# karfly/learnable-triangulation-pytorch

Measured on NVIDIA H100. Metric: volumetric samples/sec (4-view 384x384, 64^3 grid), higher is better.
Workload: dtype fp16x3 (split-fp16 operands, 3 wgmma products per term, fp32 accumulate)

## Files before the change

learnable-triangulation-pytorch_b200/csrc/common.cuh:

```cuda
#pragma once
#include <cuda_runtime.h>
#include <cuda_fp16.h>
#include <stdint.h>
#include <stdio.h>
#include <stdarg.h>
#include "../../include/lt_b200.h"

namespace lt {

char* err_buf();
int fail(int code, const char* fmt, ...);

#define LT_REQUIRE(cond, ...)                                   \
  do {                                                          \
    if (!(cond)) return ::lt::fail(LT_ERR_INVALID, __VA_ARGS__); \
  } while (0)

#define LT_CHECK_LAUNCH(name)                                                                  \
  do {                                                                                         \
    cudaError_t e__ = cudaGetLastError();                                                      \
    if (e__ != cudaSuccess) return ::lt::fail(LT_ERR_CUDA, "%s: %s", name, cudaGetErrorString(e__)); \
  } while (0)

const lt_options& opts();
int sm_count();

struct DeviceOnce {
  unsigned long long done = 0;
  bool first() {
    int dev = 0;
    if (cudaGetDevice(&dev) != cudaSuccess || dev < 0 || dev > 63) return true;
    const unsigned long long bit = 1ull << dev;
    return (__atomic_fetch_or(&done, bit, __ATOMIC_ACQ_REL) & bit) == 0;
  }
};

static inline int ceil_div(long a, long b) { return (int)((a + b - 1) / b); }

typedef __half sh_t;
constexpr float kLoScale = 1.0f;
constexpr float kLoInv = 1.0f;

__device__ __forceinline__ void split_s32(float x, sh_t& hi, sh_t& lo) {
  if (fabsf(x) <= 3.402823466e+38f) x = fminf(fmaxf(x, -65504.0f), 65504.0f);
  hi = __float2half_rn(x);
  lo = __float2half_rn((x - __half2float(hi)) * kLoScale);
}
__device__ __forceinline__ float join_s32(sh_t hi, sh_t lo) {
  return fmaf(__half2float(lo), kLoInv, __half2float(hi));
}
__device__ __host__ __forceinline__ int s32_off(int c) { return ((c >> 5) << 6) + (c & 31); }

__device__ __forceinline__ void store_s32x4(sh_t* row, int c, float4 v) {
  sh_t h[4], l[4];
  split_s32(v.x, h[0], l[0]);
  split_s32(v.y, h[1], l[1]);
  split_s32(v.z, h[2], l[2]);
  split_s32(v.w, h[3], l[3]);
  sh_t* p = row + s32_off(c);
  *reinterpret_cast<uint2*>(p) = *reinterpret_cast<uint2*>(h);
// ... 36 lines not shown
```

learnable-triangulation-pytorch_b200/csrc/conv_fold.cu:

```cuda
#include "tc_common.cuh"
#include "conv_tc_params.cuh"

namespace lt {

constexpr int kFoldThreads = 384;
constexpr int kFoldSmem = 227 * 1024;

template <int NC>
struct LinesCfg {
  static constexpr int N = 3 * NC;
  static constexpr int SLICE = N * 128;
  static constexpr int B_BYTES = 9 * SLICE;
  static constexpr int PLANE = 32 * 1024;
  static constexpr int RING = 3;
  static constexpr int XCH = 2 * 2 * 4 * 2 * 4 * (NC / 4) * 4;
  static constexpr int SLAB = 8 * 1024;
  static constexpr int A_OFF = B_BYTES;
  static constexpr int S_OFF = A_OFF + RING * PLANE;
  static constexpr int X_OFF = S_OFF + 2 * SLAB;
  static constexpr int BAR_OFF = X_OFF + XCH;
  static constexpr size_t SMEM = (size_t)BAR_OFF + 128 + 1024;
  static_assert(SLICE % 1024 == 0 && B_BYTES % 1024 == 0, "B slices must start on 1024-byte swizzle atoms");
  static_assert(SMEM <= (size_t)kFoldSmem, "shared memory");
};
// ... 67 lines not shown
  uint64_t* afull = reinterpret_cast<uint64_t*>(smem + C::BAR_OFF);
  uint64_t* aempty = afull + C::RING;
  uint64_t* bfull = aempty + C::RING;
  uint64_t* rfull = bfull + 1;
  uint64_t* rempty = rfull + 2;

  const int wg = __shfl_sync(0xffffffffu, (int)(threadIdx.x >> 7), 0);
  const int lane = threadIdx.x & 31;
  const int W = p.bw, LPB = p.bh / 2;
  const long total = (long)p.N * p.th * p.OD;
  const long q0 = (long)blockIdx.x * total / gridDim.x, q1 = (long)(blockIdx.x + 1) * total / gridDim.x;

  if (threadIdx.x == 0) {
    for (int s = 0; s < C::RING; ++s) { mbar_init(&afull[s], 1); mbar_init(&aempty[s], 256); }
    mbar_init(&bfull[0], 1);
    for (int s = 0; s < 2; ++s) { mbar_init(&rfull[s], 1); mbar_init(&rempty[s], 1); }
    fence_barrier_init();
    prefetch_tmap(&tmA);
    prefetch_tmap(&tmB);
    prefetch_tmap(&tmO);
    if (p.residual != LT_RES_NONE) prefetch_tmap(&tmR);
  }
  __syncthreads();

  if (wg == 0) {
    regs_release_producer();
    if (threadIdx.x < 32) {
      if (elect_one()) {
        mbar_expect_tx(&bfull[0], (uint32_t)C::B_BYTES);
        tma_load_3d(bsm, &tmB, &bfull[0], 0, 0, 0);
      }
      const uint32_t box_bytes = (uint32_t)((p.bh + 2) * W * 128), res_bytes = (uint32_t)(LPB * W * 128);
      int s = 0;
      uint32_t ph = 0, rph = 0;
      long q = q0;
      LinesPiece pc;
      while (lines_next_piece(p, q, q1, pc)) {
        for (int dd = pc.dA - 1; dd <= pc.dB; ++dd) {
          mbar_wait(&aempty[s], ph ^ 1u);
          if (elect_one()) {
            mbar_expect_tx(&afull[s], box_bytes);
            tma_load_5d(asm_ + (size_t)s * C::PLANE, &tmA, &afull[s], 0, 0, pc.h0 - 1, dd, pc.n);
          }
          __syncwarp();
          if (++s == C::RING) { s = 0; ph ^= 1u; }
          if (dd > pc.dA) {
            for (int r = 0; r < 2; ++r) {
              mbar_wait(&rempty[r], rph ^ 1u);
              if (elect_one()) {
                if (p.residual != LT_RES_NONE) {
                  mbar_expect_tx(&rfull[r], res_bytes);
                  tma_load_5d(ssm + (size_t)r * C::SLAB, &tmR, &rfull[r], 0, 0, pc.h0 + r * LPB, dd - 1, pc.n);
                } else {
                  mbar_arrive_local(&rfull[r]);
// ... 169 lines not shown
  int rc = make_in_map(&tmA, d, p.bw, p.bh + 2, 1, 1, in);
  if (rc) return rc;
  const uint64_t dims[3] = {64, (uint64_t)C::N, 9};
  const uint64_t str[2] = {128, (uint64_t)C::SLICE};
  const uint32_t bx[3] = {64, (uint32_t)C::N, 9};
  rc = make_map(&tmB, weight, 3, dims, str, bx, nullptr, 1);
  if (rc) return rc;
  CUtensorMap tmO, tmR;
  const int f32 = d->out_format == LT_FMT_F32;
  const uint64_t odims[5] = {(uint64_t)(f32 ? 32 : 64), (uint64_t)d->OW, (uint64_t)d->OH, (uint64_t)d->OD, (uint64_t)d->N};
  const uint64_t ostr[4] = {128, 128ull * d->OW, 128ull * d->OW * d->OH, 128ull * d->OW * d->OH * d->OD};
  const uint32_t obx[5] = {(uint32_t)(f32 ? 32 : 64), (uint32_t)d->OW, (uint32_t)(p.bh / 2), 1, 1};
  rc = make_map(&tmO, out, 5, odims, ostr, obx, nullptr, 1, f32);
  if (rc) return rc;
  rc = make_map(&tmR, residual ? residual : out, 5, odims, ostr, obx, nullptr, 1, f32);
  if (rc) return rc;
  static DeviceOnce configured;
  if (configured.first()) {
    cudaError_t e = cudaFuncSetAttribute(conv_lines_kernel<NC>, cudaFuncAttributeMaxDynamicSharedMemorySize, kFoldSmem);
    if (e != cudaSuccess) return fail(LT_ERR_CUDA, "conv_lines: cudaFuncSetAttribute: %s", cudaGetErrorString(e));
  }
  const long planes = (long)p.N * p.th * p.OD;
  const int grid = (int)(planes < sm_count() ? planes : sm_count());
  conv_lines_kernel<NC><<<grid, kFoldThreads, C::SMEM, st>>>(tmA, tmB, tmO, tmR, p);
  cudaError_t e = cudaGetLastError();
  if (e != cudaSuccess) return fail(LT_ERR_CUDA, "conv_lines_kernel: %s", cudaGetErrorString(e));
  return LT_OK;
}

template <int K, int NC>
struct FoldCfg {
  static_assert(K == 7, "the 3^3 layers run on conv_lines_kernel");
  static constexpr int BW = 8, BH = 16, BD = 2;
  static constexpr int WBOX = BW + K - 1, HBOX = BH + K - 1, DBOX = BD;
  static constexpr int A_BYTES = WBOX * HBOX * DBOX * 128;
  static constexpr int ASTAGES = K;
  static constexpr int TAP = NC * 128;
  static constexpr int B_SLICE = K * TAP;
  static constexpr int MB = 2;
  static constexpr int AVAIL = kFoldSmem - 1024 - 256;
  static constexpr int ARING = 2;
  static constexpr int BRING_FIT = (AVAIL - ARING * A_BYTES) / B_SLICE;
  static constexpr int BRING = BRING_FIT > 4 ? 4 : BRING_FIT;
  static constexpr int A_OFF = BRING * B_SLICE;
  static constexpr int BAR_OFF = A_OFF + ARING * A_BYTES;
  static constexpr size_t SMEM = (size_t)BAR_OFF + 256 + 1024;
  static_assert(BW * BH * BD == 256 && BH % 8 == 0, "two m64 blocks of whole 8-wide lines per warpgroup");
  static_assert(A_BYTES % 1024 == 0 && B_SLICE % 1024 == 0, "boxes must start on 1024-byte swizzle atoms");
// ... 35 lines not shown
                                                                    const __grid_constant__ CUtensorMap tmB, const TcParams p) {
  using C = FoldCfg<K, NC>;
  extern __shared__ uint8_t smem_raw[];
  uint8_t* smem = reinterpret_cast<uint8_t*>((reinterpret_cast<uintptr_t>(smem_raw) + 1023) & ~(uintptr_t)1023);
  uint8_t* bsm = smem;
  uint8_t* asm_ = smem + C::A_OFF;
  uint64_t* afull = reinterpret_cast<uint64_t*>(smem + C::BAR_OFF);
  uint64_t* aempty = afull + C::ARING;
  uint64_t* bfull = aempty + C::ARING;
  uint64_t* bempty = bfull + C::BRING;

  const int wg = __shfl_sync(0xffffffffu, (int)(threadIdx.x >> 7), 0);
  const int lane = threadIdx.x & 31;
  const int ntiles = p.tw * p.th * p.td * p.tn;

  if (threadIdx.x == 0) {
    for (int s = 0; s < C::ARING; ++s) { mbar_init(&afull[s], 1); mbar_init(&aempty[s], 256); }
    for (int s = 0; s < C::BRING; ++s) { mbar_init(&bfull[s], 1); mbar_init(&bempty[s], 2); }
    fence_barrier_init();
    prefetch_tmap(&tmA);
    prefetch_tmap(&tmB);
  }
  __syncthreads();

  if (wg == 0) {
    regs_release_producer();
    if (threadIdx.x < 32) {
      int sa = 0, sb = 0;
      uint32_t pa = 0, pb = 0;
      for (int t = blockIdx.x; t < ntiles; t += gridDim.x) {
        int ow0, oh0, od0, nb;
        fold_tile_origin(p, t, ow0, oh0, od0, nb);
        for (int as = 0; as < C::ASTAGES; ++as) {
          mbar_wait(&aempty[sa], pa ^ 1u);
          if (elect_one()) {
            mbar_expect_tx(&afull[sa], (uint32_t)C::A_BYTES);
            tma_load_5d(asm_ + (size_t)sa * C::A_BYTES, &tmA, &afull[sa], 0, ow0 - K / 2, oh0 - K / 2, od0 + as - K / 2, nb);
          }
          __syncwarp();
          if (++sa == C::ARING) { sa = 0; pa ^= 1u; }
          for (int kw = 0; kw < K; ++kw) {
            mbar_wait(&bempty[sb], pb ^ 1u);
            if (elect_one()) {
              mbar_expect_tx(&bfull[sb], (uint32_t)C::B_SLICE);
              tma_load_3d(bsm + (size_t)sb * C::B_SLICE, &tmB, &bfull[sb], 0, 0, (kw * K + as) * K);
            }
            __syncwarp();
            if (++sb == C::BRING) { sb = 0; pb ^= 1u; }
          }
        }
      }
    }
    return;
  }

  regs_claim_consumer();
  const int g = wg - 1, warp = (threadIdx.x >> 5) & 3;
  float d1[C::MB][NC / 2], d2[C::MB][NC / 2];
#pragma unroll
  for (int b = 0; b < C::MB; ++b)
#pragma unroll
    for (int i = 0; i < NC / 2; ++i) { d1[b][i] = 0.f; d2[b][i] = 0.f; }
  int blk_dd[C::MB], blk_hb[C::MB];
  uint32_t row0[C::MB];
#pragma unroll
  for (int b = 0; b < C::MB; ++b) {
    const int blk = C::MB * g + b;
    blk_dd[b] = blk / (C::BH / 8);
    blk_hb[b] = blk % (C::BH / 8);
    row0[b] = (uint32_t)((blk_dd[b] * C::HBOX + blk_hb[b] * 8 + 2 * warp) * C::WBOX + (lane & 7));
  }
  const uint32_t mlane = (uint32_t)(lane >> 3);
  const int r_lo = warp * 16 + (lane >> 2);
  const int c2 = 2 * (lane & 3);
  const uint32_t bsm0 = smem_u32(bsm), asm0 = smem_u32(asm_);
  const bool wg_lead = (threadIdx.x & 127) == 0;
  int bprev = -1;
  for (int kt = 0;; ++kt) {
    const int t = blockIdx.x + kt * gridDim.x;
    if (t >= ntiles) break;
#pragma unroll 1
    for (int as = 0; as < C::ASTAGES; ++as) {
      const int na = kt * C::ASTAGES + as;
      const int sa = na % C::ARING;
      mbar_wait(&afull[sa], (uint32_t)(na / C::ARING) & 1u);
      const uint32_t box = asm0 + (uint32_t)(sa * C::A_BYTES);
#pragma unroll 1
      for (int kw = 0; kw < K; ++kw) {
        const int nbs = na * K + kw;
        const int sb = nbs % C::BRING;
        mbar_wait(&bfull[sb], (uint32_t)(nbs / C::BRING) & 1u);
        const uint32_t bslice = bsm0 + (uint32_t)(sb * C::B_SLICE);
        uint32_t ln[K + 1][C::MB][2][4];
#pragma unroll
        for (int b = 0; b < C::MB; ++b) fold_load_line(ln[0][b], box, row0[b] + kw, mlane);
#pragma unroll
        for (int kh = 0; kh < K; ++kh) {
#pragma unroll
          for (int b = 0; b < C::MB; ++b) fold_load_line(ln[kh + 1][b], box, row0[b] + kw + (uint32_t)((kh + 1) * C::WBOX), mlane);
          wg_fence();
          const uint64_t bd = make_sw128_desc(bslice + (uint32_t)(kh * C::TAP));
          const uint32_t acc = (as == 0 && kw == 0 && kh == 0) ? 0u : 1u;
#pragma unroll
// ... 40 lines not shown
                         const void* residual, void* out, cudaStream_t st) {
  constexpr int K = 7;
  using C = FoldCfg<K, NC>;
  TcParams p;
  fill_params(d, p, 1, NC, NC, 3, scale, shift, residual, out);
  p.bw = C::BW; p.bh = C::BH; p.bd = C::BD; p.bn = 1;
  p.tw = ceil_div(d->OW, p.bw); p.th = ceil_div(d->OH, p.bh); p.td = ceil_div(d->OD, p.bd); p.tn = d->N;
  p.stages = C::ARING;
  CUtensorMap tmA, tmB;
  int rc = make_in_map(&tmA, d, C::WBOX, C::HBOX, C::DBOX, 1, in);
  if (rc) return rc;
  const uint64_t dims[3] = {64, (uint64_t)NC, (uint64_t)K * K * K};
  const uint64_t str[2] = {128, (uint64_t)NC * 128};
  const uint32_t bx[3] = {64, (uint32_t)NC, (uint32_t)K};
  rc = make_map(&tmB, weight, 3, dims, str, bx, nullptr, 1);
  if (rc) return rc;
  static DeviceOnce configured;
  if (configured.first()) {
    cudaError_t e = cudaFuncSetAttribute(conv_fold_kernel<K, NC>, cudaFuncAttributeMaxDynamicSharedMemorySize, kFoldSmem);
    if (e != cudaSuccess) return fail(LT_ERR_CUDA, "conv_fold: cudaFuncSetAttribute: %s", cudaGetErrorString(e));
  }
  const long ntiles = (long)p.tw * p.th * p.td * p.tn;
  const int grid = (int)(ntiles < sm_count() ? ntiles : sm_count());
  conv_fold_kernel<K, NC><<<grid, kFoldThreads, C::SMEM, st>>>(tmA, tmB, p);
  cudaError_t e = cudaGetLastError();
  if (e != cudaSuccess) return fail(LT_ERR_CUDA, "conv_fold_kernel: %s", cudaGetErrorString(e));
  return LT_OK;
}

int conv_fold_supported(const lt_conv_desc* d) {
  const bool cubic = d->KD == d->KH && d->KH == d->KW && (d->KW == 3 || d->KW == 7);
  const int pd = d->KW / 2;
  return cubic && d->Cin == 32 && d->Cout <= 32 && d->sd == 1 && d->sh == 1 && d->sw == 1 && d->pd == pd && d->ph == pd &&
         d->pw == pd && d->OD == d->ID && d->OH == d->IH && d->OW == d->IW && d->osd == 1 && d->osh == 1 && d->osw == 1 &&
         d->ood == 0 && d->ooh == 0 && d->oow == 0 && d->FD == d->OD && d->FH == d->OH && d->FW == d->OW && d->FC == 32 &&
         d->in_format == LT_FMT_S32 && d->IW >= 16 && (d->KW == 7 || d->IW <= 64);
}

int conv_fold_fwd(const lt_conv_desc* d, const void* in, const void* weight, const float* scale, const float* shift,
                  const void* residual, void* out, void* stream) {
  LT_REQUIRE(conv_fold_supported(d), "conv_fold: unsupported layer shape");
  const cudaStream_t st = (cudaStream_t)stream;
  const bool narrow = d->Cout <= 16;
  if (d->KW == 3)
    return narrow ? conv_lines_run<16>(d, in, weight, scale, shift, residual, out, st)
                  : conv_lines_run<32>(d, in, weight, scale, shift, residual, out, st);
  return narrow ? conv_fold_run<16>(d, in, weight, scale, shift, residual, out, st)
                : conv_fold_run<32>(d, in, weight, scale, shift, residual, out, st);
// ... 42 lines not shown
```

learnable-triangulation-pytorch_b200/csrc/conv_tail.cu:

```cuda
#include "conv_tc_params.cuh"
#include "softargmax_common.cuh"

namespace lt {

struct TailParams {
  const float* scale1; const float* shift1;
  const float* scale2; const float* shift2;
  const float* scale3; const float* bias3;
  float* logits;
  long rows;
  long tiles;
  int FC;
  const float* coord;
  float* partial;
  int B, J, tiles_per_sample, softmax;
  float mult;
};

constexpr int kTailThreads = 384;
constexpr int kTailStages = 2;
constexpr int kTailWBytes = 32 * 128;
constexpr int kTailHBytes = 64 * 128;
constexpr int kTailOffH = kTailStages * kATileBytes;
constexpr int kTailOffW = kTailOffH + 2 * kTailHBytes;
// ... 44 lines not shown
  }
}

template <int STATS>
__global__ void __launch_bounds__(kTailThreads, 2) v2v_tail_kernel(const __grid_constant__ CUtensorMap tmX,
                                                                    const __grid_constant__ CUtensorMap tmW1,
                                                                    const __grid_constant__ CUtensorMap tmW2,
                                                                    const __grid_constant__ CUtensorMap tmW3, const TailParams p) {
  extern __shared__ uint8_t smem_raw[];
  uint8_t* smem = reinterpret_cast<uint8_t*>((reinterpret_cast<uintptr_t>(smem_raw) + 1023) & ~(uintptr_t)1023);
  uint8_t* w_tiles = smem + kTailOffW;
  uint64_t* a_full = reinterpret_cast<uint64_t*>(smem + kTailOffBar);
  uint64_t* a_empty = a_full + kTailStages;
  uint64_t* w_full = a_empty + kTailStages;

  const int wg = __shfl_sync(0xffffffffu, (int)(threadIdx.x >> 7), 0);
  const int lane = threadIdx.x & 31;
  if (threadIdx.x == 0) {
    for (int s = 0; s < kTailStages; ++s) { mbar_init(&a_full[s], 1); mbar_init(&a_empty[s], 2); }
    mbar_init(w_full, 1);
    fence_barrier_init();
  }
  __syncthreads();

  if (wg == 0) {
    if (threadIdx.x < 32) {
      if (elect_one()) {
        prefetch_tmap(&tmX);
        mbar_expect_tx(w_full, 3u * kTailWBytes);
        tma_load_2d(w_tiles, &tmW1, w_full, 0, 0);
        tma_load_2d(w_tiles + kTailWBytes, &tmW2, w_full, 0, 0);
        tma_load_2d(w_tiles + 2 * kTailWBytes, &tmW3, w_full, 0, 0);
      }
      __syncwarp();
      uint32_t s = 0, ph = 0;
      for (long t = blockIdx.x; t < p.tiles; t += gridDim.x) {
        mbar_wait(&a_empty[s], ph ^ 1u);
        if (elect_one()) {
          mbar_expect_tx(&a_full[s], (uint32_t)kATileBytes);
          tma_load_2d(smem + s * kATileBytes, &tmX, &a_full[s], 0, (int)(t * 128));
        }
        __syncwarp();
        if (++s == kTailStages) { s = 0; ph ^= 1u; }
      }
    }
    return;
  }

  const int g = wg - 1;
  const int wq = (threadIdx.x >> 5) & 3;
  const int rl = wq * 16 + (lane >> 2);
  const int c2 = 2 * (lane & 3);
  const uint32_t hbase = smem_u32(smem + kTailOffH + g * kTailHBytes);
  const uint64_t hd = make_sw128_desc(hbase);
  const uint64_t w1 = make_sw128_desc(smem_u32(w_tiles)), w2 = make_sw128_desc(smem_u32(w_tiles + kTailWBytes)),
                 w3 = make_sw128_desc(smem_u32(w_tiles + 2 * kTailWBytes));
  constexpr bool SM = STATS == 1;
// ... 17 lines not shown
        SoftState t{o[0], o[1], o[2], o[3], o[4]};
        st_merge(a, t, SM);
      }
      float* dst = p.partial + (((long)b * gridDim.x + blockIdx.x) * p.J + lane) * 5;
      dst[0] = a.m; dst[1] = a.d; dst[2] = a.sx; dst[3] = a.sy; dst[4] = a.sz;
    }
    tail_consumers_sync();
  };
  if (STATS) {
    for (int i = threadIdx.x - 128; i < p.B * p.J; i += 256) {
      const int b = i / p.J, j = i % p.J;
      const long lo = (long)b * p.tiles_per_sample, G = gridDim.x;
      const long f0 = lo + (((long)blockIdx.x - lo) % G + G) % G;
      if (!(f0 < lo + p.tiles_per_sample)) {
        float* dst = p.partial + (((long)b * G + blockIdx.x) * p.J + j) * 5;
        dst[0] = SM ? -INFINITY : 0.0f; dst[1] = 0.f; dst[2] = 0.f; dst[3] = 0.f; dst[4] = 0.f;
      }
    }
  }

  mbar_wait(w_full, 0);
  uint32_t s = 0, ph = 0;
  for (long t = blockIdx.x; t < p.tiles; t += gridDim.x) {
    if (STATS) {
      const int b = (int)(t / p.tiles_per_sample);
      if (b != cur_b) {
        if (cur_b >= 0) flush(cur_b);
        cur_b = b;
      }
    }
    float d[16];
    mbar_wait(&a_full[s], ph);
    gemm32(d, make_sw128_desc(smem_u32(smem + s * kATileBytes + g * kTailHBytes)), w1);
    if ((threadIdx.x & 127) == 0) mbar_arrive_local(&a_empty[s]);
    if (++s == kTailStages) { s = 0; ph ^= 1u; }
#pragma unroll
    for (int layer = 0; layer < 2; ++layer) {
      tail_wg_sync(g);
      hidden_store(d, layer == 0 ? p.scale1 : p.scale2, layer == 0 ? p.shift1 : p.shift2, hbase, rl, c2);
      fence_proxy_async();
      tail_wg_sync(g);
      gemm32(d, hd, layer == 0 ? w2 : w3);
    }
#pragma unroll
    for (int h = 0; h < 2; ++h) {
      const int rw = (lane >> 2) + 8 * h;
// ... 50 lines not shown
    if (rc) return rc;
  }
  const void* ws[3] = {w1, w2, w3};
  const uint64_t wrows[3] = {32, 32, (uint64_t)((p.FC + 15) & ~15)};
  for (int i = 0; i < 3; ++i) {
    const uint64_t dims[2] = {64, wrows[i]};
    const uint64_t str[1] = {128};
    const uint32_t bx[2] = {64, 32};
    int rc = make_map(&tmW[i], ws[i], 2, dims, str, bx, nullptr, 1);
    if (rc) return rc;
  }
  p.tiles = (p.rows + 127) / 128;
  static DeviceOnce configured;
  if (configured.first()) {
    cudaError_t e = cudaFuncSetAttribute(v2v_tail_kernel<0>, cudaFuncAttributeMaxDynamicSharedMemorySize, kTailSmem);
    if (e == cudaSuccess) e = cudaFuncSetAttribute(v2v_tail_kernel<1>, cudaFuncAttributeMaxDynamicSharedMemorySize, kTailSmemStats);
    if (e == cudaSuccess) e = cudaFuncSetAttribute(v2v_tail_kernel<2>, cudaFuncAttributeMaxDynamicSharedMemorySize, kTailSmemStats);
    if (e != cudaSuccess) return fail(LT_ERR_CUDA, "v2v_tail: cudaFuncSetAttribute: %s", cudaGetErrorString(e));
  }
  long grid = 2L * sm_count();
  if (grid > p.tiles) grid = p.tiles;
  if (grid_out) *grid_out = (int)grid;
  cudaStream_t st = (cudaStream_t)stream;
  if (stats == 1) v2v_tail_kernel<1><<<(unsigned)grid, kTailThreads, kTailSmemStats, st>>>(tmX, tmW[0], tmW[1], tmW[2], p);
  else if (stats == 2) v2v_tail_kernel<2><<<(unsigned)grid, kTailThreads, kTailSmemStats, st>>>(tmX, tmW[0], tmW[1], tmW[2], p);
  else v2v_tail_kernel<0><<<(unsigned)grid, kTailThreads, kTailSmem, st>>>(tmX, tmW[0], tmW[1], tmW[2], p);
  LT_CHECK_LAUNCH("v2v_tail_kernel");
  return LT_OK;
}

extern "C" int lt_v2v_tail_fwd(const void* x, const void* w1, const void* w2, const void* w3, const float* scale1, const float* shift1,
                               const float* scale2, const float* shift2, const float* scale3, const float* bias3, float* logits, long rows,
                               int FC, void* stream) {
  LT_REQUIRE(x && w1 && w2 && w3 && scale1 && shift1 && scale2 && shift2 && scale3 && bias3 && logits, "v2v_tail: null pointer");
  LT_REQUIRE(rows > 0 && rows < (1L << 31) && FC % 4 == 0 && FC >= 4 && FC <= 32, "v2v_tail: bad sizes (rows=%ld FC=%d)", rows, FC);
  TailParams p;
  p.scale1 = scale1; p.shift1 = shift1; p.scale2 = scale2; p.shift2 = shift2; p.scale3 = scale3; p.bias3 = bias3;
  p.logits = logits; p.rows = rows; p.FC = FC;
  p.coord = nullptr; p.partial = nullptr; p.B = 0; p.J = 0; p.tiles_per_sample = 1; p.softmax = 0; p.mult = 1.0f;
  return launch_tail(x, w1, w2, w3, p, 0, nullptr, stream);
}

extern "C" int lt_v2v_tail_stats_fwd(const void* x, const void* w1, const void* w2, const void* w3, const float* scale1, const float* shift1,
                                     const float* scale2, const float* shift2, const float* scale3, const float* bias3, float* logits, int B,
                                     long nvox, int FC, const float* coord, int J, float multiplier, int softmax, void* workspace,
                                     size_t workspace_bytes, int* n_partials, void* stream) {
  LT_REQUIRE(x && w1 && w2 && w3 && scale1 && shift1 && scale2 && shift2 && scale3 && bias3 && logits && coord && workspace && n_partials,
             "v2v_tail_stats: null pointer");
  LT_REQUIRE(B > 0 && nvox > 0 && nvox % 128 == 0 && (long)B * nvox < (1L << 31), "v2v_tail_stats: bad sizes (B=%d nvox=%ld)", B, nvox);
  LT_REQUIRE(FC % 4 == 0 && FC >= 4 && FC <= kTailStatMaxFC && J > 0 && J <= FC, "v2v_tail_stats: need J <= FC <= %d, FC %% 4 == 0", kTailStatMaxFC);
// ... 12 lines not shown
```

learnable-triangulation-pytorch_b200/csrc/conv_tc.cu:

```cuda
#include "tc_common.cuh"
#include "conv_tc_params.cuh"
#include <stdlib.h>
#include <string.h>

namespace lt {

constexpr int kTcThreads = 384;

struct TcUnit {
  int m, n0, z, q_begin, nchunks;
};
__device__ __forceinline__ TcUnit tc_unit(const TcParams& p, int u, int m_tiles, int nchunks_all) {
  TcUnit w;
  const int n = u % p.n_tiles;
  u /= p.n_tiles;
  w.m = u % m_tiles;
  w.z = u / m_tiles;
  w.n0 = n * p.Nt;
  w.q_begin = (int)(((long)w.z * nchunks_all) / p.splits);
  w.nchunks = (int)(((long)(w.z + 1) * nchunks_all) / p.splits) - w.q_begin;
  return w;
}
__device__ __forceinline__ void tc_tile_origin(const TcParams& p, int t, int& ow0, int& oh0, int& od0, int& nb0) {
  ow0 = (t % p.tw) * p.bw; t /= p.tw;
// ... 25 lines not shown
  const int epi_bytes = tc_epi_bytes(NT, p.splits);
  const bool staged = epi_bytes > 0;
  uint8_t* ebuf = smem + (size_t)p.stages * kStage;
  uint64_t* full = reinterpret_cast<uint64_t*>(ebuf + epi_bytes);
  uint64_t* empty = full + p.stages;
  uint64_t* efull = empty + p.stages;
  uint64_t* edone = efull + 1;

  const int wg = __shfl_sync(0xffffffffu, (int)(threadIdx.x >> 7), 0);
  const int lane = threadIdx.x & 31;
  const int m_tiles = p.tw * p.th * p.td * p.tn;
  const int units = m_tiles * p.n_tiles * p.splits;
  const int nchunks_all = p.KD * p.KH * p.KW * p.CB;

  if (threadIdx.x == 0) {
    for (int s = 0; s < p.stages; ++s) { mbar_init(&full[s], 1); mbar_init(&empty[s], 2); }
    mbar_init(efull, 1);
    mbar_init(edone, 256);
    fence_barrier_init();
    prefetch_tmap(&tmA);
    prefetch_tmap(&tmB);
  }
  __syncthreads();

  if (wg == 0) {
    regs_release_producer();
    if (staged && threadIdx.x == 32) {
      uint32_t eph = 0;
      for (int u = blockIdx.x; u < units; u += gridDim.x) {
        const TcUnit w = tc_unit(p, u, m_tiles, nchunks_all);
        int ow0, oh0, od0, nb0;
        tc_tile_origin(p, w.m, ow0, oh0, od0, nb0);
        bulk_wait_read0();
        if (p.residual != LT_RES_NONE) {
          mbar_expect_tx(efull, (uint32_t)epi_bytes);
          for (int sl = 0; sl < NT / 32; ++sl) {
            int g, c;
            epi_slab(p, w.n0 + 32 * sl, g, c);
            tma_load_5d(ebuf + sl * kSlabBytes, &tmE.res[g], efull, c, ow0, oh0, od0, nb0);
          }
        } else {
          mbar_arrive_local(efull);
        }
        mbar_wait(edone, eph);
        eph ^= 1u;
        for (int sl = 0; sl < NT / 32; ++sl) {
          int g, c;
          epi_slab(p, w.n0 + 32 * sl, g, c);
          tma_store_5d(&tmE.out[g], ebuf + sl * kSlabBytes, c, ow0, oh0, od0, nb0);
        }
        bulk_commit();
      }
      bulk_wait0();
    }
    if (threadIdx.x < 32) {
      int s = 0;
      uint32_t ph = 0;
      for (int u = blockIdx.x; u < units; u += gridDim.x) {
        const TcUnit w = tc_unit(p, u, m_tiles, nchunks_all);
        int ow0, oh0, od0, nb0;
        tc_tile_origin(p, w.m, ow0, oh0, od0, nb0);
        int tap = w.q_begin / p.CB, cb = w.q_begin - tap * p.CB;
        int kw = tap % p.KW, kh = (tap / p.KW) % p.KH, kd = tap / (p.KW * p.KH);
        const int ax = ow0 * p.sw - p.pw, ay = oh0 * p.sh - p.ph, az = od0 * p.sd - p.pd, bn0 = w.n0 * p.b_nmul;
        for (int q = 0, qa = w.q_begin; q < w.nchunks; ++q, ++qa) {
          mbar_wait(&empty[s], ph ^ 1u);
          uint8_t* a_dst = smem + (size_t)s * kStage;
          if (elect_one()) {
            mbar_expect_tx(&full[s], (uint32_t)kStage);
            tma_load_5d(a_dst, &tmA, &full[s], cb * 64, ax + kw, ay + kh, az + kd, nb0);
            tma_load_2d(a_dst + kATileBytes, &tmB, &full[s], qa * p.b_step0, qa * p.b_step1 + bn0);
          }
          __syncwarp();
          if (++cb == p.CB) { cb = 0; if (++kw == p.KW) { kw = 0; if (++kh == p.KH) { kh = 0; ++kd; } } }
          if (++s == p.stages) { s = 0; ph ^= 1u; }
        }
      }
    }
    return;
  }

  regs_claim_consumer();
  const int g = wg - 1;
  float d1[NT / 2], d2[NT / 2];
#pragma unroll
  for (int i = 0; i < NT / 2; ++i) { d1[i] = 0.f; d2[i] = 0.f; }
  const int r0 = g * 64 + ((threadIdx.x >> 5) & 3) * 16 + (lane >> 2);
  const int c2 = 2 * (lane & 3);
  const uint32_t ring0 = smem_u32(smem);
  int s = 0;
  uint32_t ph = 0, eph = 0;
  for (int u = blockIdx.x; u < units; u += gridDim.x) {
    const TcUnit w = tc_unit(p, u, m_tiles, nchunks_all);
    int prev = -1;
    for (int q = 0; q < w.nchunks; ++q) {
      mbar_wait(&full[s], ph);
      const uint32_t a_addr = ring0 + (uint32_t)(s * kStage) + (uint32_t)(g * 64 * 128);
      const uint32_t b_addr = ring0 + (uint32_t)(s * kStage) + kATileBytes;
      const uint64_t ad = make_sw128_desc(a_addr), bd = make_sw128_desc(b_addr);
      const uint32_t acc = (q == 0) ? 0u : 1u;
      wg_fence();
      if (p.terms == 3) {
        wgmma_f16<NT>(d1, ad, bd, acc);
        wgmma_f16<NT>(d1, ad + 2, bd + 2, 1u);
        wgmma_f16<NT>(d2, ad, bd + 4, acc);
        wgmma_f16<NT>(d2, ad + 2, bd + 6, 1u);
        wgmma_f16<NT>(d2, ad + 4, bd, 1u);
        wgmma_f16<NT>(d2, ad + 6, bd + 2, 1u);
      } else if (p.terms == 1) {
        wgmma_f16<NT>(d1, ad, bd, acc);
        wgmma_f16<NT>(d1, ad + 2, bd + 2, 1u);
      } else {
        wgmma_f16<NT>(d1, ad, bd, acc);
        wgmma_f16<NT>(d1, ad + 2, bd + 2, 1u);
        wgmma_f16<NT>(d1, ad + 4, bd + 4, 1u);
// ... 165 lines not shown
  slot.used = true;
  slot.key = key;
  slot.map = *map;
  return LT_OK;
}

static int pow2_ceil(int v) { int p = 1; while (p < v) p <<= 1; return p; }

static void pick_box(int OW, int OH, int OD, int N, int* box) {
  double best = 1e300;
  for (int bw = 1; bw <= 128; bw <<= 1)
    for (int bh = 1; bw * bh <= 128; bh <<= 1)
      for (int bd = 1; bw * bh * bd <= 128; bd <<= 1) {
        const int bn = 128 / (bw * bh * bd);
        if (bw > pow2_ceil(OW) || bh > pow2_ceil(OH) || bd > pow2_ceil(OD) || bn > pow2_ceil(N)) continue;
        const double padded = (double)ceil_div(OW, bw) * bw * ceil_div(OH, bh) * bh * (double)ceil_div(OD, bd) * bd * ceil_div(N, bn) * bn;
        const double score = padded * (1.0 + 1e-3 / bw);
        if (score < best) { best = score; box[0] = bw; box[1] = bh; box[2] = bd; box[3] = bn; }
      }
  if (best == 1e300) { box[0] = pow2_ceil(OW) > 128 ? 128 : pow2_ceil(OW); box[1] = box[2] = 1; box[3] = 128 / box[0]; }
}

__global__ void __launch_bounds__(256) splitk_reduce_kernel(const TcParams p, long m_tiles, int coutp) {
  const int c4 = coutp >> 2;
  const long total = m_tiles * 128 * c4;
  for (long i = (long)blockIdx.x * blockDim.x + threadIdx.x; i < total; i += (long)gridDim.x * blockDim.x) {
    const int co = (int)(i % c4) * 4;
    const long tr = i / c4;
    const int row = (int)(tr % 128);
    long t = tr / 128;
    const int twi = (int)(t % p.tw); t /= p.tw;
    const int thi = (int)(t % p.th); t /= p.th;
    const int tdi = (int)(t % p.td); t /= p.td;
    const int tni = (int)t;
    int r_ = row;
    const int dw = r_ % p.bw; r_ /= p.bw;
    const int dh = r_ % p.bh; r_ /= p.bh;
    const int dd = r_ % p.bd; r_ /= p.bd;
    const int ow = twi * p.bw + dw, oh = thi * p.bh + dh, od = tdi * p.bd + dd, nb = tni * p.bn + r_;
    if (!(ow < p.OW && oh < p.OH && od < p.OD && nb < p.N) || co >= p.FC) continue;
    const long opix = (((long)nb * p.FD + (od * p.osd + p.ood)) * p.FH + (oh * p.osh + p.ooh)) * p.FW + (ow * p.osw + p.oow);
    float4 a = make_float4(0.f, 0.f, 0.f, 0.f);
    for (int z = 0; z < p.splits; ++z) {
      const float4 v = *reinterpret_cast<const float4*>(p.ws + ((size_t)z * m_tiles * 128 + tr) * p.ws_ld + co);
      a.x += v.x; a.y += v.y; a.z += v.z; a.w += v.w;
    }
// ... 13 lines not shown
    else store_s32x4(reinterpret_cast<sh_t*>(p.out) + opix * 2 * p.FC, co, o);
  }
}

static int out_groups(const lt_conv_desc* d) {
  const int g = (d->ogd > 1 ? d->ogd : 1) * (d->ogh > 1 ? d->ogh : 1) * (d->ogw > 1 ? d->ogw : 1);
  return g;
}

static int pick_nt(int CoutP) {
  for (int nt = 128; nt > 16; nt >>= 1)
    if (CoutP % nt == 0) return nt;
  return 16;
}

template <int NT>
static int launch_nt(const CUtensorMap& tmA, const CUtensorMap& tmB, const TcEpiMaps& tmE, const TcParams& p, dim3 grid, size_t smem,
                     cudaStream_t st) {
  static DeviceOnce configured;
  if (configured.first()) {
    cudaError_t e = cudaFuncSetAttribute(conv_tc_kernel<NT>, cudaFuncAttributeMaxDynamicSharedMemorySize, (int)(227 * 1024));
    if (e != cudaSuccess) return fail(LT_ERR_CUDA, "conv_tc: cudaFuncSetAttribute: %s", cudaGetErrorString(e));
  }
  conv_tc_kernel<NT><<<grid, kTcThreads, smem, st>>>(tmA, tmB, tmE, p);
  cudaError_t e = cudaGetLastError();
  if (e != cudaSuccess) return fail(LT_ERR_CUDA, "conv_tc_kernel: %s", cudaGetErrorString(e));
  return LT_OK;
}

static double tc_model_clocks(long tiles, int chunks, int nt, int splits, int sm) {
  const long units = tiles * splits;
  const long grid = units < sm ? units : sm;
  const long waves = (units + grid - 1) / grid;
  const double chunk = fmax(12.0 * 64.0 * nt / 128.0, (kATileBytes + nt * 128.0) / 30.0);
  const double epilogue = 128.0 * nt * 4.0 / 30.0;
  double t = (double)waves * ((double)ceil_div(chunks, splits) * chunk + epilogue);
  if (splits > 1) t += 7000.0 + (double)tiles * 128 * nt * 4.0 * (splits + 2) / 1500.0;
  return t;
}

static void tc_plan(long m_tiles, int n_tiles, int nt, int chunks, int terms, int n_maps, int splitk, size_t ws_bytes, int sm,
                    int* splits_out, int* grid_out) {
  const long tiles = m_tiles * n_tiles;
  int best = 1;
  if (splitk && terms != 0 && n_maps == 1) {
    const size_t per_split = (size_t)tiles * 128 * nt * sizeof(float);
    double best_t = tc_model_clocks(tiles, chunks, nt, 1, sm);
    for (int s = 2; s <= chunks / 4 && (size_t)s * per_split <= ws_bytes; ++s) {
      const double t = tc_model_clocks(tiles, chunks, nt, s, sm);
// ... 49 lines not shown
  const int epi_bytes = tc_epi_bytes(p.Nt, splits);
  int stages = (kTcSmemBudget - epi_bytes) / stage_bytes;
  if (stages > 8) stages = 8;
  p.stages = stages;
  const size_t smem = (size_t)stages * stage_bytes + epi_bytes + (2 * stages + 2) * 8 + 1024;
  TcEpiMaps tmE{};
  int rc;
  if (epi_bytes) {
    rc = make_epi_maps(p, &tmE);
    if (rc) return rc;
  }
  switch (p.Nt) {
    case 128: rc = launch_nt<128>(tmA, tmB, tmE, p, dim3(grid), smem, st); break;
    case 64: rc = launch_nt<64>(tmA, tmB, tmE, p, dim3(grid), smem, st); break;
    case 32: rc = launch_nt<32>(tmA, tmB, tmE, p, dim3(grid), smem, st); break;
    case 16: rc = launch_nt<16>(tmA, tmB, tmE, p, dim3(grid), smem, st); break;
    default: return fail(LT_ERR_INVALID, "conv_tc: unsupported N tile %d", p.Nt);
  }
  if (rc) return rc;
  if (splits > 1) {
    const long total = m_tiles * 128 * (p.ws_ld / 4);
    long blocks = (total + 255) / 256;
    if (blocks > 4L * sm_count()) blocks = 4L * sm_count();
    splitk_reduce_kernel<<<(unsigned)blocks, 256, 0, st>>>(p, m_tiles, p.ws_ld);
    cudaError_t e = cudaGetLastError();
    if (e != cudaSuccess) return fail(LT_ERR_CUDA, "splitk_reduce_kernel: %s", cudaGetErrorString(e));
  }
  return LT_OK;
}

void fill_params(const lt_conv_desc* d, TcParams& p, int CB, int CoutP, int Nt, int terms, const float* scale, const float* shift,
                        const void* residual, void* out) {
  p.OW = d->OW; p.OH = d->OH; p.OD = d->OD; p.N = d->N;
  int box[4];
  pick_box(d->OW, d->OH, d->OD, d->N, box);
  p.bw = box[0]; p.bh = box[1]; p.bd = box[2]; p.bn = box[3];
  p.tw = ceil_div(d->OW, p.bw); p.th = ceil_div(d->OH, p.bh); p.td = ceil_div(d->OD, p.bd); p.tn = ceil_div(d->N, p.bn);
  p.KW = d->KW; p.KH = d->KH; p.KD = d->KD; p.pw = d->pw; p.ph = d->ph; p.pd = d->pd;
  p.sw = d->sw; p.sh = d->sh; p.sd = d->sd;
  p.CB = CB; p.b_step0 = 0; p.b_step1 = CoutP; p.b_nmul = 1; p.Nt = Nt; p.terms = terms;
  p.FC = d->FC; p.FD = d->FD; p.FH = d->FH; p.FW = d->FW;
  p.osd = d->osd; p.osh = d->osh; p.osw = d->osw; p.ood = d->ood; p.ooh = d->ooh; p.oow = d->oow;
  p.relu = d->relu; p.residual = d->residual; p.out_format = d->out_format;
  p.scale = scale; p.shift = shift; p.res = residual; p.out = out;
  p.splits = 1; p.ws = nullptr; p.ws_ld = 0; p.ws_gain = 1.0f; p.stages = 0; p.n_tiles = 1;
  p.n_maps = out_groups(d);
  p.oc = p.n_maps > 1 ? d->Cout / p.n_maps : CoutP;
  p.gh = d->ogh > 1 ? d->ogh : 1; p.gw = d->ogw > 1 ? d->ogw : 1;
}
// ... 142 lines not shown
```

Baseline: 206.9.

## Launch conv kernels with PDL and prefetch weights before grid dependency wait

Switches the conv_lines, conv_fold, conv_tc, v2v tail and split-K reduce launches to programmatic dependent launch. Each kernel issues its weight (B) TMA loads before griddepcontrol.wait and triggers its dependents near its last tile. This lets one kernel's prologue and weight fetch overlap the previous kernel's tail, hiding launch gaps across a chain of many small conv layers. The risk is subtle barrier and transaction accounting: the producer must skip B loads that were already issued, and an early trigger could race if any dependent touches data before its wait.

```diff
diff --git a/learnable-triangulation-pytorch_b200/csrc/common.cuh b/learnable-triangulation-pytorch_b200/csrc/common.cuh
--- a/learnable-triangulation-pytorch_b200/csrc/common.cuh
+++ b/learnable-triangulation-pytorch_b200/csrc/common.cuh
@@ -4,6 +4,7 @@
 #include <stdint.h>
 #include <stdio.h>
 #include <stdarg.h>
+#include <utility>
 #include "../../include/lt_b200.h"
 
 namespace lt {
@@ -36,6 +37,29 @@
 };
 
 static inline int ceil_div(long a, long b) { return (int)((a + b - 1) / b); }
+
+__device__ __forceinline__ void pdl_wait() { asm volatile("griddepcontrol.wait;" ::: "memory"); }
+__device__ __forceinline__ void pdl_trigger() { asm volatile("griddepcontrol.launch_dependents;" ::: "memory"); }
+
+template <typename... KArgs, typename... Args>
+static inline cudaError_t launch_pdl(void (*kernel)(KArgs...), dim3 grid, dim3 block, size_t smem, cudaStream_t st, Args&&... args) {
+  cudaLaunchAttribute attr[1];
+  attr[0].id = cudaLaunchAttributeProgrammaticStreamSerialization;
+  attr[0].val.programmaticStreamSerializationAllowed = 1;
+  cudaLaunchConfig_t cfg = {};
+  cfg.gridDim = grid;
+  cfg.blockDim = block;
+  cfg.dynamicSmemBytes = smem;
+  cfg.stream = st;
+  cfg.attrs = attr;
+  cfg.numAttrs = 1;
+  return cudaLaunchKernelEx(&cfg, kernel, std::forward<Args>(args)...);
+}
+#define LT_CHECK_PDL(name, call)                                                                \
+  do {                                                                                          \
+    cudaError_t e__ = (call);                                                                   \
+    if (e__ != cudaSuccess) return ::lt::fail(LT_ERR_CUDA, "%s: %s", name, cudaGetErrorString(e__)); \
+  } while (0)
 
 typedef __half sh_t;
 constexpr float kLoScale = 1.0f;
diff --git a/learnable-triangulation-pytorch_b200/csrc/conv_fold.cu b/learnable-triangulation-pytorch_b200/csrc/conv_fold.cu
--- a/learnable-triangulation-pytorch_b200/csrc/conv_fold.cu
+++ b/learnable-triangulation-pytorch_b200/csrc/conv_fold.cu
@@ -113,14 +113,19 @@
     if (p.residual != LT_RES_NONE) prefetch_tmap(&tmR);
   }
   __syncthreads();
+  if (threadIdx.x < 32) {
+    if (elect_one()) {
+      mbar_expect_tx(&bfull[0], (uint32_t)C::B_BYTES);
+      tma_load_3d(bsm, &tmB, &bfull[0], 0, 0, 0);
+    }
+    __syncwarp();
+  }
+  pdl_wait();
+  pdl_trigger();
 
   if (wg == 0) {
     regs_release_producer();
     if (threadIdx.x < 32) {
-      if (elect_one()) {
-        mbar_expect_tx(&bfull[0], (uint32_t)C::B_BYTES);
-        tma_load_3d(bsm, &tmB, &bfull[0], 0, 0, 0);
-      }
       const uint32_t box_bytes = (uint32_t)((p.bh + 2) * W * 128), res_bytes = (uint32_t)(LPB * W * 128);
       int s = 0;
       uint32_t ph = 0, rph = 0;
@@ -336,8 +341,7 @@
   }
   const long planes = (long)p.N * p.th * p.OD;
   const int grid = (int)(planes < sm_count() ? planes : sm_count());
-  conv_lines_kernel<NC><<<grid, kFoldThreads, C::SMEM, st>>>(tmA, tmB, tmO, tmR, p);
-  cudaError_t e = cudaGetLastError();
+  cudaError_t e = launch_pdl(conv_lines_kernel<NC>, grid, dim3(kFoldThreads), C::SMEM, st, tmA, tmB, tmO, tmR, p);
   if (e != cudaSuccess) return fail(LT_ERR_CUDA, "conv_lines_kernel: %s", cudaGetErrorString(e));
   return LT_OK;
 }
@@ -419,6 +423,18 @@
     prefetch_tmap(&tmB);
   }
   __syncthreads();
+  constexpr int kBPre = C::BRING < C::ASTAGES * K ? C::BRING : C::ASTAGES * K;
+  if (threadIdx.x < 32 && (int)blockIdx.x < ntiles) {
+    if (elect_one()) {
+      for (int i = 0; i < kBPre; ++i) {
+        const int as = i / K, kw = i % K;
+        mbar_expect_tx(&bfull[i], (uint32_t)C::B_SLICE);
+        tma_load_3d(bsm + (size_t)i * C::B_SLICE, &tmB, &bfull[i], 0, 0, (kw * K + as) * K);
+      }
+    }
+    __syncwarp();
+  }
+  pdl_wait();
 
   if (wg == 0) {
     regs_release_producer();
@@ -438,7 +454,7 @@
           if (++sa == C::ARING) { sa = 0; pa ^= 1u; }
           for (int kw = 0; kw < K; ++kw) {
             mbar_wait(&bempty[sb], pb ^ 1u);
-            if (elect_one()) {
+            if (!(t == (int)blockIdx.x && as * K + kw < kBPre) && elect_one()) {
               mbar_expect_tx(&bfull[sb], (uint32_t)C::B_SLICE);
               tma_load_3d(bsm + (size_t)sb * C::B_SLICE, &tmB, &bfull[sb], 0, 0, (kw * K + as) * K);
             }
@@ -476,6 +492,7 @@
   for (int kt = 0;; ++kt) {
     const int t = blockIdx.x + kt * gridDim.x;
     if (t >= ntiles) break;
+    if (t + (int)gridDim.x >= ntiles) pdl_trigger();
 #pragma unroll 1
     for (int as = 0; as < C::ASTAGES; ++as) {
       const int na = kt * C::ASTAGES + as;
@@ -562,8 +579,7 @@
   }
   const long ntiles = (long)p.tw * p.th * p.td * p.tn;
   const int grid = (int)(ntiles < sm_count() ? ntiles : sm_count());
-  conv_fold_kernel<K, NC><<<grid, kFoldThreads, C::SMEM, st>>>(tmA, tmB, p);
-  cudaError_t e = cudaGetLastError();
+  cudaError_t e = launch_pdl(conv_fold_kernel<K, NC>, grid, dim3(kFoldThreads), C::SMEM, st, tmA, tmB, p);
   if (e != cudaSuccess) return fail(LT_ERR_CUDA, "conv_fold_kernel: %s", cudaGetErrorString(e));
   return LT_OK;
 }
diff --git a/learnable-triangulation-pytorch_b200/csrc/conv_tail.cu b/learnable-triangulation-pytorch_b200/csrc/conv_tail.cu
--- a/learnable-triangulation-pytorch_b200/csrc/conv_tail.cu
+++ b/learnable-triangulation-pytorch_b200/csrc/conv_tail.cu
@@ -90,17 +90,20 @@
     fence_barrier_init();
   }
   __syncthreads();
+  if (threadIdx.x < 32) {
+    if (elect_one()) {
+      prefetch_tmap(&tmX);
+      mbar_expect_tx(w_full, 3u * kTailWBytes);
+      tma_load_2d(w_tiles, &tmW1, w_full, 0, 0);
+      tma_load_2d(w_tiles + kTailWBytes, &tmW2, w_full, 0, 0);
+      tma_load_2d(w_tiles + 2 * kTailWBytes, &tmW3, w_full, 0, 0);
+    }
+    __syncwarp();
+  }
+  pdl_wait();
 
   if (wg == 0) {
     if (threadIdx.x < 32) {
-      if (elect_one()) {
-        prefetch_tmap(&tmX);
-        mbar_expect_tx(w_full, 3u * kTailWBytes);
-        tma_load_2d(w_tiles, &tmW1, w_full, 0, 0);
-        tma_load_2d(w_tiles + kTailWBytes, &tmW2, w_full, 0, 0);
-        tma_load_2d(w_tiles + 2 * kTailWBytes, &tmW3, w_full, 0, 0);
-      }
-      __syncwarp();
       uint32_t s = 0, ph = 0;
       for (long t = blockIdx.x; t < p.tiles; t += gridDim.x) {
         mbar_wait(&a_empty[s], ph ^ 1u);
@@ -164,6 +167,7 @@
   mbar_wait(w_full, 0);
   uint32_t s = 0, ph = 0;
   for (long t = blockIdx.x; t < p.tiles; t += gridDim.x) {
+    if (t + gridDim.x >= p.tiles) pdl_trigger();
     if (STATS) {
       const int b = (int)(t / p.tiles_per_sample);
       if (b != cur_b) {
@@ -260,10 +264,12 @@
   if (grid > p.tiles) grid = p.tiles;
   if (grid_out) *grid_out = (int)grid;
   cudaStream_t st = (cudaStream_t)stream;
-  if (stats == 1) v2v_tail_kernel<1><<<(unsigned)grid, kTailThreads, kTailSmemStats, st>>>(tmX, tmW[0], tmW[1], tmW[2], p);
-  else if (stats == 2) v2v_tail_kernel<2><<<(unsigned)grid, kTailThreads, kTailSmemStats, st>>>(tmX, tmW[0], tmW[1], tmW[2], p);
-  else v2v_tail_kernel<0><<<(unsigned)grid, kTailThreads, kTailSmem, st>>>(tmX, tmW[0], tmW[1], tmW[2], p);
-  LT_CHECK_LAUNCH("v2v_tail_kernel");
+  const dim3 g((unsigned)grid), b(kTailThreads);
+  cudaError_t e;
+  if (stats == 1) e = launch_pdl(v2v_tail_kernel<1>, g, b, kTailSmemStats, st, tmX, tmW[0], tmW[1], tmW[2], p);
+  else if (stats == 2) e = launch_pdl(v2v_tail_kernel<2>, g, b, kTailSmemStats, st, tmX, tmW[0], tmW[1], tmW[2], p);
+  else e = launch_pdl(v2v_tail_kernel<0>, g, b, kTailSmem, st, tmX, tmW[0], tmW[1], tmW[2], p);
+  LT_CHECK_PDL("v2v_tail_kernel", e);
   return LT_OK;
 }
 
diff --git a/learnable-triangulation-pytorch_b200/csrc/conv_tc.cu b/learnable-triangulation-pytorch_b200/csrc/conv_tc.cu
--- a/learnable-triangulation-pytorch_b200/csrc/conv_tc.cu
+++ b/learnable-triangulation-pytorch_b200/csrc/conv_tc.cu
@@ -71,6 +71,20 @@
     prefetch_tmap(&tmB);
   }
   __syncthreads();
+  int b_pre = 0;
+  if (threadIdx.x < 32 && (int)blockIdx.x < units) {
+    const TcUnit w = tc_unit(p, blockIdx.x, m_tiles, nchunks_all);
+    b_pre = w.nchunks < p.stages ? w.nchunks : p.stages;
+    if (elect_one()) {
+      for (int q = 0; q < b_pre; ++q) {
+        const int qa = w.q_begin + q;
+        mbar_expect_tx(&full[q], (uint32_t)kStage);
+        tma_load_2d(smem + (size_t)q * kStage + kATileBytes, &tmB, &full[q], qa * p.b_step0, qa * p.b_step1 + w.n0 * p.b_nmul);
+      }
+    }
+    __syncwarp();
+  }
+  pdl_wait();
 
   if (wg == 0) {
     regs_release_producer();
@@ -116,9 +130,10 @@
           mbar_wait(&empty[s], ph ^ 1u);
           uint8_t* a_dst = smem + (size_t)s * kStage;
           if (elect_one()) {
-            mbar_expect_tx(&full[s], (uint32_t)kStage);
+            const bool b_issued = (int)u == (int)blockIdx.x && q < b_pre;
+            if (!b_issued) mbar_expect_tx(&full[s], (uint32_t)kStage);
             tma_load_5d(a_dst, &tmA, &full[s], cb * 64, ax + kw, ay + kh, az + kd, nb0);
-            tma_load_2d(a_dst + kATileBytes, &tmB, &full[s], qa * p.b_step0, qa * p.b_step1 + bn0);
+            if (!b_issued) tma_load_2d(a_dst + kATileBytes, &tmB, &full[s], qa * p.b_step0, qa * p.b_step1 + bn0);
           }
           __syncwarp();
           if (++cb == p.CB) { cb = 0; if (++kw == p.KW) { kw = 0; if (++kh == p.KH) { kh = 0; ++kd; } } }
@@ -140,6 +155,7 @@
   int s = 0;
   uint32_t ph = 0, eph = 0;
   for (int u = blockIdx.x; u < units; u += gridDim.x) {
+    if (u + (int)gridDim.x >= units) pdl_trigger();
     const TcUnit w = tc_unit(p, u, m_tiles, nchunks_all);
     int prev = -1;
     for (int q = 0; q < w.nchunks; ++q) {
@@ -351,6 +367,8 @@
 }
 
 __global__ void __launch_bounds__(256) splitk_reduce_kernel(const TcParams p, long m_tiles, int coutp) {
+  pdl_wait();
+  pdl_trigger();
   const int c4 = coutp >> 2;
   const long total = m_tiles * 128 * c4;
   for (long i = (long)blockIdx.x * blockDim.x + threadIdx.x; i < total; i += (long)gridDim.x * blockDim.x) {
@@ -410,9 +428,7 @@
     cudaError_t e = cudaFuncSetAttribute(conv_tc_kernel<NT>, cudaFuncAttributeMaxDynamicSharedMemorySize, (int)(227 * 1024));
     if (e != cudaSuccess) return fail(LT_ERR_CUDA, "conv_tc: cudaFuncSetAttribute: %s", cudaGetErrorString(e));
   }
-  conv_tc_kernel<NT><<<grid, kTcThreads, smem, st>>>(tmA, tmB, tmE, p);
-  cudaError_t e = cudaGetLastError();
-  if (e != cudaSuccess) return fail(LT_ERR_CUDA, "conv_tc_kernel: %s", cudaGetErrorString(e));
+  LT_CHECK_PDL("conv_tc_kernel", launch_pdl(conv_tc_kernel<NT>, grid, dim3(kTcThreads), smem, st, tmA, tmB, tmE, p));
   return LT_OK;
 }
 
@@ -508,9 +524,7 @@
     const long total = m_tiles * 128 * (p.ws_ld / 4);
     long blocks = (total + 255) / 256;
     if (blocks > 4L * sm_count()) blocks = 4L * sm_count();
-    splitk_reduce_kernel<<<(unsigned)blocks, 256, 0, st>>>(p, m_tiles, p.ws_ld);
-    cudaError_t e = cudaGetLastError();
-    if (e != cudaSuccess) return fail(LT_ERR_CUDA, "splitk_reduce_kernel: %s", cudaGetErrorString(e));
+    LT_CHECK_PDL("splitk_reduce_kernel", launch_pdl(splitk_reduce_kernel, dim3((unsigned)blocks), dim3(256), 0, st, p, m_tiles, p.ws_ld));
   }
   return LT_OK;
 }
```

Result: no change. 205.9 (median of 6 runs) (-0.5%).
